# Oscar-W-Chen/gpu-ai-inference-server

Measured on AMD Instinct MI355X. Metric: images/sec, DenseNet-121 fp32, batch 32 per GPU, device-resident inputs, higher is better.
Workload: dtype f32; 1 GPU; DenseNet-121 fp32 batch=32 per GPU, synthetic 3x224x224 inputs (BASELINE configs[1]); synthetic ONNX graph + seeded random weights (reference model file is not in the mount); global_batch=32, per_gpu_batch=32, parallelism=dp1 (independent batch shards)

## Files before the change

gpu-ai-inference-server_amd/csrc/kernels_direct.hip:

```cpp
#include <hip/hip_runtime.h>

#include <algorithm>
#include <cstdlib>

#include "env.h"
#include "kernels.h"

namespace ie {

typedef float f32x16 __attribute__((ext_vector_type(16)));
typedef float f32x4 __attribute__((ext_vector_type(4)));
typedef float f32x2 __attribute__((ext_vector_type(2)));
typedef unsigned u32x4 __attribute__((ext_vector_type(4)));
typedef _Float16 h8 __attribute__((ext_vector_type(8)));
typedef _Float16 h2 __attribute__((ext_vector_type(2)));

struct DirectGeom {
    int cpt;
    int total;
};

template <bool HALF, int TN, int WAVES, int MAXC, bool PRE>
__global__ __launch_bounds__(64 * WAVES) void conv_direct_kernel(const ConvArgs a, const DirectGeom g) {
    constexpr int NT = 64 * WAVES, BN = 32 * TN;
    constexpr int CW = HALF ? 32 : 16;
    constexpr int ESZ = HALF ? 2 : 4;
    constexpr int PP = BN + 4;
    constexpr unsigned OOB = 0x80000000u;
    extern __shared__ __attribute__((aligned(16))) unsigned char smem_direct[];
    float* const sPart = reinterpret_cast<float*>(smem_direct);
    unsigned char* const sPre = smem_direct + size_t(WAVES) * 32 * PP * 4;

    const int tid = threadIdx.x, lane = tid & 63, r = lane & 31, hh = lane >> 5;
    const int wave = __builtin_amdgcn_readfirstlane(tid >> 6);
    const int Cin = a.in.c, H = a.in.h, W = a.in.w, OH = a.out.h, OW = a.out.w, Cout = a.out.c;
    const int M = a.out.n * OH * OW;
    const int m0 = blockIdx.x * 32, n0 = blockIdx.y * BN;
    const int KK = a.kh * a.kw;

    const int m = m0 + r;
    const bool mok = m < M;
    const int mm = mok ? m : 0;
    const int b = mm / (OH * OW);
    const int rem = mm - b * (OH * OW);
    const int oy = rem / OW, ox = rem - oy * OW;
    const int iy0 = oy * a.sh - a.pt, ix0 = ox * a.sw - a.pl;

    const int cb = int(int64_t(g.total) * wave / WAVES), ce = int(int64_t(g.total) * (wave + 1) / WAVES);
    const __amdgpu_buffer_rsrc_t rs_in = __builtin_amdgcn_make_buffer_rsrc(a.in.p, 0, int(a.in_bytes), 0x00020000);
    const void* const wbase = HALF ? a.w16 : static_cast<const void*>(a.w);
    const __amdgpu_buffer_rsrc_t rs_w = __builtin_amdgcn_make_buffer_rsrc(const_cast<void*>(wbase), 0, Cout * KK * Cin * ESZ, 0x00020000);

    u32x4 A[MAXC][2], B[MAXC][TN][2];
    unsigned okmask = 0;
#pragma unroll
    for (int i = 0; i < MAXC; ++i) {
        const int ch = cb + i;
        const bool live = ch < ce;
        const int chc = live ? ch : cb;
        const int tap = chc / g.cpt, c0 = (chc - tap * g.cpt) * CW;
        const int ky = tap / a.kw, kx = tap - ky * a.kw;
        const int iy = iy0 + ky, ix = ix0 + kx;
        const bool ok = live && mok && unsigned(iy) < unsigned(H) && unsigned(ix) < unsigned(W);
        okmask |= ok ? (1u << i) : 0u;
        const unsigned offA = ok ? unsigned(int(b * a.in.sn + iy * a.in.sh + ix * a.in.sw) + c0 + hh * (CW / 4)) * unsigned(ESZ) : OOB;
        A[i][0] = __builtin_amdgcn_raw_buffer_load_b128(rs_in, offA, 0, 0);
        A[i][1] = __builtin_amdgcn_raw_buffer_load_b128(rs_in, offA + unsigned(CW / 2 * ESZ), 0, 0);
#pragma unroll
        for (int j = 0; j < TN; ++j) {
            const int n = n0 + j * 32 + r;
            const unsigned offB = (live && n < Cout) ? unsigned((n * KK + tap) * Cin + c0 + hh * (CW / 4)) * unsigned(ESZ) : OOB;
            B[i][j][0] = __builtin_amdgcn_raw_buffer_load_b128(rs_w, offB, 0, 0);
            B[i][j][1] = __builtin_amdgcn_raw_buffer_load_b128(rs_w, offB + unsigned(CW / 2 * ESZ), 0, 0);
        }
    }

    if constexpr (PRE) {
        if constexpr (HALF) {
            const u32x4* const ps = static_cast<const u32x4*>(a.pre_scale16);
            const u32x4* const pt = static_cast<const u32x4*>(a.pre_shift16);
            u32x4* const ds = reinterpret_cast<u32x4*>(sPre);
            u32x4* const dt = reinterpret_cast<u32x4*>(sPre + Cin * 2);
            for (int i = tid; i < Cin / 8; i += NT) { ds[i] = ps[i]; dt[i] = pt[i]; }
        } else {
            const u32x4* const ps = reinterpret_cast<const u32x4*>(a.pre_scale);
            const u32x4* const pt = reinterpret_cast<const u32x4*>(a.pre_shift);
            u32x4* const ds = reinterpret_cast<u32x4*>(sPre);
            u32x4* const dt = reinterpret_cast<u32x4*>(sPre + Cin * 4);
            for (int i = tid; i < Cin / 4; i += NT) { ds[i] = ps[i]; dt[i] = pt[i]; }
        }
        __syncthreads();
    }

    f32x16 acc[TN];
#pragma unroll
    for (int j = 0; j < TN; ++j)
#pragma unroll
        for (int e = 0; e < 16; ++e) acc[j][e] = 0.f;

#pragma unroll
    for (int i = 0; i < MAXC; ++i) {
        if (cb + i < ce) {
            const int ch = cb + i;
            const int tap = ch / g.cpt, c0 = (ch - tap * g.cpt) * CW;
            const bool ok = (okmask >> i) & 1u;
#pragma unroll
            for (int q = 0; q < 2; ++q) {
                if constexpr (HALF) {
                    h8 av = __builtin_bit_cast(h8, A[i][q]);
                    if constexpr (PRE) {
                        const h8 s = *reinterpret_cast<const h8*>(sPre + (c0 + q * 16 + hh * 8) * 2);
                        const h8 t = *reinterpret_cast<const h8*>(sPre + Cin * 2 + (c0 + q * 16 + hh * 8) * 2);
                        av = av * s + t;
                        if (a.pre_relu) av = __builtin_elementwise_max(av, h8{});
                        if (!ok) av = h8{};
                    }
#pragma unroll
                    for (int j = 0; j < TN; ++j)
                        acc[j] = __builtin_amdgcn_mfma_f32_32x32x16_f16(__builtin_bit_cast(h8, B[i][j][q]), av, acc[j], 0, 0, 0);
                } else {
                    f32x4 av = __builtin_bit_cast(f32x4, A[i][q]);
                    if constexpr (PRE) {
                        const f32x4 s = *reinterpret_cast<const f32x4*>(sPre + (c0 + q * 8 + hh * 4) * 4);
                        const f32x4 t = *reinterpret_cast<const f32x4*>(sPre + Cin * 4 + (c0 + q * 8 + hh * 4) * 4);
#pragma unroll
                        for (int e = 0; e < 4; ++e) {
                            const float x = av[e] * s[e] + t[e];
                            av[e] = ok ? (a.pre_relu ? fmaxf(x, 0.f) : x) : 0.f;
                        }
                    }
#pragma unroll
                    for (int j = 0; j < TN; ++j) {
                        const f32x4 bv = __builtin_bit_cast(f32x4, B[i][j][q]);
#pragma unroll
                        for (int e = 0; e < 4; ++e) acc[j] = __builtin_amdgcn_mfma_f32_32x32x2f32(bv[e], av[e], acc[j], 0, 0, 0);
                    }
                }
            }
        }
    }

    float* const mine = sPart + (wave * 32 + r) * PP;
#pragma unroll
    for (int j = 0; j < TN; ++j)
#pragma unroll
        for (int gq = 0; gq < 4; ++gq)
            *reinterpret_cast<f32x4*>(mine + j * 32 + 8 * gq + 4 * hh) = f32x4{acc[j][4 * gq], acc[j][4 * gq + 1], acc[j][4 * gq + 2], acc[j][4 * gq + 3]};
    __syncthreads();
    const int esz = a.out.f16 ? 2 : 4;
    const __amdgpu_buffer_rsrc_t rs_out =
        __builtin_amdgcn_make_buffer_rsrc(a.out.p, 0, int((int64_t(M - 1) * a.out.sw + Cout) * esz), 0x00020000);
    for (int idx = tid; idx < 32 * (BN / 2); idx += NT) {
        const int p = idx / (BN / 2), c2 = (idx - p * (BN / 2)) * 2;
        f32x2 v = {0.f, 0.f};
#pragma unroll
        for (int w = 0; w < WAVES; ++w) {
            const f32x2 x = *reinterpret_cast<const f32x2*>(sPart + (w * 32 + p) * PP + c2);
            v[0] += x[0];
            v[1] += x[1];
        }
        const int n = n0 + c2;
        if (a.bias != nullptr) {
            v[0] += a.bias[n < Cout ? n : Cout - 1];
            v[1] += a.bias[n + 1 < Cout ? n + 1 : Cout - 1];
        }
        if (a.relu) { v[0] = fmaxf(v[0], 0.f); v[1] = fmaxf(v[1], 0.f); }
        const bool pok = m0 + p < M;
        const unsigned rowoff = pok ? unsigned((m0 + p) * int(a.out.sw) * esz) : OOB;
        if (a.out.f16) {
            const h2 hv = {_Float16(v[0]), _Float16(v[1])};
            __builtin_amdgcn_raw_buffer_store_b32(__builtin_bit_cast(unsigned, hv), rs_out, n < Cout ? rowoff + unsigned(n * 2) : OOB, 0, 0);
        } else {
            __builtin_amdgcn_raw_buffer_store_b64(__builtin_bit_cast(__attribute__((ext_vector_type(2))) unsigned, v), rs_out,
                                                  n < Cout ? rowoff + unsigned(n * 4) : OOB, 0, 0);
        }
    }
}

template <int TN, int WAVES, int MAXC, bool PRE>
__global__ __launch_bounds__(64 * WAVES) void conv_win_kernel(const ConvArgs a, const DirectGeom g) {
    constexpr int NT = 64 * WAVES, BN = 16 * TN, PP = BN + 4;
    constexpr unsigned OOB = 0x80000000u;
    extern __shared__ __attribute__((aligned(16))) unsigned char smem_direct[];
    float* const sWin = reinterpret_cast<float*>(smem_direct);
    float* const sPart = reinterpret_cast<float*>(smem_direct);

    const int tid = threadIdx.x, lane = tid & 63, r = lane & 15, gk = lane >> 4;
    const int wave = __builtin_amdgcn_readfirstlane(tid >> 6);
    const int Cin = a.in.c, H = a.in.h, W = a.in.w, Cout = a.out.c;
    const int P = Cin + 4;
    const int M = a.out.n * H * W;
    const int m0 = blockIdx.x * 16, n0 = blockIdx.y * BN;
    const int ipitch = int(a.in.sw);

    const int cb = int(int64_t(g.total) * wave / WAVES), ce = int(int64_t(g.total) * (wave + 1) / WAVES);
    const __amdgpu_buffer_rsrc_t rs_w =
        __builtin_amdgcn_make_buffer_rsrc(const_cast<float*>(a.wfrag), 0, Cout * a.kh * a.kw * Cin * 4, 0x00020000);
    u32x4 B[MAXC][TN];
#pragma unroll
    for (int i = 0; i < MAXC; ++i) {
        const int ch = cb + i;
#pragma unroll
        for (int j = 0; j < TN; ++j)
            B[i][j] = __builtin_amdgcn_raw_buffer_load_b128(
                rs_w, ch < ce ? unsigned(((int(blockIdx.y) * TN + j) * g.total + ch) * 64 + lane) * 16u : OOB, 0, 0);
    }

    {
        constexpr int U = 4;
        const __amdgpu_buffer_rsrc_t rs_in = __builtin_amdgcn_make_buffer_rsrc(a.in.p, 0, int(a.in_bytes), 0x00020000);
        const int c4n = Cin >> 2;
        const int p_lo = m0 - a.pt * W - a.pl;
        const int npx = 16 + (a.kh - 1) * W + (a.kw - 1);
        const int items = npx * c4n;
        for (int idx0 = tid; idx0 < items; idx0 += U * NT) {
            u32x4 v[U];
            int row[U], c4[U];
#pragma unroll
            for (int u = 0; u < U; ++u) {
                const int idx = idx0 + u * NT;
                row[u] = idx / c4n;
                c4[u] = idx - row[u] * c4n;
                const int p = p_lo + row[u];
                v[u] = __builtin_amdgcn_raw_buffer_load_b128(rs_in, (idx < items && p >= 0 && p < M) ? unsigned(p * ipitch + c4[u] * 4) * 4u : OOB, 0, 0);
            }
#pragma unroll
            for (int u = 0; u < U; ++u) {
                if (idx0 + u * NT < items) {
                    f32x4 x = __builtin_bit_cast(f32x4, v[u]);
                    if constexpr (PRE) {
                        const f32x4 sc = *reinterpret_cast<const f32x4*>(a.pre_scale + c4[u] * 4);
                        const f32x4 sf = *reinterpret_cast<const f32x4*>(a.pre_shift + c4[u] * 4);
#pragma unroll
                        for (int e = 0; e < 4; ++e) {
                            const float y = x[e] * sc[e] + sf[e];
                            x[e] = a.pre_relu ? fmaxf(y, 0.f) : y;
                        }
                    }
                    *reinterpret_cast<f32x4*>(sWin + row[u] * P + c4[u] * 4) = x;
                }
            }
        }
    }
    __syncthreads();

    const int m = m0 + r;
    const bool mok = m < M;
    const int rem = (mok ? m : 0) % (H * W);
    const int oy = rem / W, ox = rem - oy * W;

    f32x4 acc[TN];
#pragma unroll
    for (int j = 0; j < TN; ++j) acc[j] = f32x4{0.f, 0.f, 0.f, 0.f};
#pragma unroll
    for (int i = 0; i < MAXC; ++i) {
        if (cb + i < ce) {
            const int ch = cb + i;
            const int tap = ch / g.cpt, c0 = (ch - tap * g.cpt) * 16;
            const int ky = tap / a.kw, kx = tap - ky * a.kw;
            const bool ok = mok && unsigned(oy + ky - a.pt) < unsigned(H) && unsigned(ox + kx - a.pl) < unsigned(W);
            f32x4 av = *reinterpret_cast<const f32x4*>(sWin + (r + ky * W + kx) * P + c0 + gk * 4);
            if (!ok) av = f32x4{0.f, 0.f, 0.f, 0.f};
#pragma unroll
            for (int j = 0; j < TN; ++j) {
                const f32x4 bv = __builtin_bit_cast(f32x4, B[i][j]);
#pragma unroll
                for (int e = 0; e < 4; ++e) acc[j] = __builtin_amdgcn_mfma_f32_16x16x4f32(bv[e], av[e], acc[j], 0, 0, 0);
            }
        }
    }
    __syncthreads();

#pragma unroll
    for (int j = 0; j < TN; ++j) *reinterpret_cast<f32x4*>(sPart + (wave * 16 + r) * PP + j * 16 + 4 * gk) = acc[j];
    __syncthreads();
    const __amdgpu_buffer_rsrc_t rs_out =
        __builtin_amdgcn_make_buffer_rsrc(a.out.p, 0, int((int64_t(M - 1) * a.out.sw + Cout) * 4), 0x00020000);
    for (int idx = tid; idx < 16 * (BN / 2); idx += NT) {
        const int p = idx / (BN / 2), c2 = (idx - p * (BN / 2)) * 2;
        f32x2 v = {0.f, 0.f};
#pragma unroll
        for (int w = 0; w < WAVES; ++w) {
            const f32x2 x = *reinterpret_cast<const f32x2*>(sPart + (w * 16 + p) * PP + c2);
            v[0] += x[0];
            v[1] += x[1];
        }
        const int n = n0 + c2;
        if (a.bias != nullptr) { v[0] += a.bias[n]; v[1] += a.bias[n + 1]; }
        if (a.relu) { v[0] = fmaxf(v[0], 0.f); v[1] = fmaxf(v[1], 0.f); }
        __builtin_amdgcn_raw_buffer_store_b64(__builtin_bit_cast(__attribute__((ext_vector_type(2))) unsigned, v), rs_out,
                                              m0 + p < M ? unsigned((m0 + p) * int(a.out.sw) + n) * 4u : OOB, 0, 0);
    }
}

__global__ __launch_bounds__(256) void permute_weights_frag_kernel(const float* __restrict__ src, float* __restrict__ dst, int Cout, int KK, int Cin) {
    const int cpt = Cin >> 4, total = KK * cpt;
    const int64_t n4 = int64_t(Cout) * KK * Cin / 4;
    for (int64_t i = int64_t(blockIdx.x) * 256 + threadIdx.x; i < n4; i += int64_t(gridDim.x) * 256) {
        const int lane = int(i & 63);
        const int64_t t = i >> 6;
        const int ch = int(t % total), nb = int(t / total);
        const int tap = ch / cpt, c0 = (ch - tap * cpt) * 16;
        const int r = lane & 15, gk = lane >> 4;
        reinterpret_cast<f32x4*>(dst)[i] = *reinterpret_cast<const f32x4*>(src + (int64_t(nb * 16 + r) * KK + tap) * Cin + c0 + gk * 4);
    }
}

hipError_t LaunchPermuteWeightsFrag(const float* src, float* dst, int Cout, int KK, int Cin, hipStream_t stream) {
    if ((Cout % 16) || (Cin % 16) || Cout <= 0 || KK <= 0) return hipErrorInvalidValue;
    const int64_t n4 = int64_t(Cout) * KK * Cin / 4;
    const unsigned blocks = unsigned(std::min<int64_t>((n4 + 255) / 256, 2048));
    permute_weights_frag_kernel<<<dim3(blocks), dim3(256), 0, stream>>>(src, dst, Cout, KK, Cin);
    return hipGetLastError();
}

struct WinTile { int tn, waves, maxc; };
constexpr int kNumWinTiles = 4;
constexpr WinTile kWinTiles[kNumWinTiles] = {{1, 8, 9}, {2, 8, 9}, {1, 4, 18}, {2, 4, 18}};

static size_t win_lds_bytes(const ConvArgs& a, const WinTile& t) {
    const size_t win = size_t(16 + (a.kh - 1) * a.in.w + (a.kw - 1)) * (a.in.c + 4) * 4;
    const size_t part = size_t(t.waves) * 16 * (16 * t.tn + 4) * 4;
    return win > part ? win : part;
}

static bool win_eligible(const ConvArgs& a, int wt) {
    const WinTile t = kWinTiles[wt];
    if (a.in.f16 || a.out.f16 || a.wfrag == nullptr || a.res.p != nullptr) return false;
    if (a.in.sc != 1 || a.out.sc != 1 || (a.in.c % 16) || (a.out.c % (16 * t.tn))) return false;
    if (a.sh != 1 || a.sw != 1 || a.out.h != a.in.h || a.out.w != a.in.w || a.out.n != a.in.n) return false;
    if (a.pt < 0 || a.pl < 0 || a.pt >= a.kh || a.pl >= a.kw) return false;
    if ((a.in.sw % 4) || a.in.sh != a.in.w * a.in.sw || a.in.sn != a.in.h * a.in.sh || (reinterpret_cast<uintptr_t>(a.in.p) & 15)) return false;
    if ((reinterpret_cast<uintptr_t>(a.wfrag) & 15) || (a.out.sw & 1) || (reinterpret_cast<uintptr_t>(a.out.p) & 7)) return false;
    if (a.out.sh != a.out.w * a.out.sw || a.out.sn != a.out.h * a.out.sh) return false;
    if (a.pre_scale && ((reinterpret_cast<uintptr_t>(a.pre_scale) & 15) || (reinterpret_cast<uintptr_t>(a.pre_shift) & 15))) return false;
    const int64_t M = int64_t(a.out.n) * a.out.h * a.out.w;
    if (M > 65536 || (M + 64) * a.in.sw * 4 >= (int64_t(1) << 31) || M * a.out.sw * 4 >= (int64_t(1) << 31) ||
        int64_t(a.out.c) * a.kh * a.kw * a.in.c * 4 >= (int64_t(1) << 31))
        return false;
    const int total = a.kh * a.kw * (a.in.c / 16);
    if (total > t.waves * t.maxc || total < t.waves) return false;
    return win_lds_bytes(a, t) <= size_t(160) * 1024;
}

template <int WT>
static hipError_t launch_win_t(const ConvArgs& a, hipStream_t stream) {
    constexpr WinTile t = kWinTiles[WT];
    DirectGeom g;
    g.cpt = a.in.c / 16;
    g.total = a.kh * a.kw * g.cpt;
    const int64_t M = int64_t(a.out.n) * a.out.h * a.out.w;
    const dim3 grid(unsigned((M + 15) / 16), unsigned(a.out.c / (16 * t.tn)));
    const size_t lds = win_lds_bytes(a, t);
    if (a.pre_scale) conv_win_kernel<t.tn, t.waves, t.maxc, true><<<grid, dim3(64 * t.waves), lds, stream>>>(a, g);
    else conv_win_kernel<t.tn, t.waves, t.maxc, false><<<grid, dim3(64 * t.waves), lds, stream>>>(a, g);
    return hipGetLastError();
}

template <int WAVES, int TNW, int PB, bool PRE>
__global__ __launch_bounds__(64 * WAVES) void conv1x1_as_kernel(const ConvArgs a) {
    constexpr int NT = 64 * WAVES, D = PB == 1 ? 16 : 8, BNW = 16 * TNW, BN = BNW * WAVES;
    constexpr unsigned OOB = 0x80000000u;
    extern __shared__ __attribute__((aligned(16))) unsigned char smem_direct[];
    float* const sA = reinterpret_cast<float*>(smem_direct);

    const int tid = threadIdx.x, lane = tid & 63, r = lane & 15, gk = lane >> 4;
    const int wave = __builtin_amdgcn_readfirstlane(tid >> 6);
    const int K = a.in.c, P = K + (a.debug >> 8), CH = K >> 4, Cout = a.out.c;
    const int M = a.out.n * a.out.h * a.out.w;
    const int m0 = blockIdx.x * (16 * PB), n0 = blockIdx.y * BN + wave * BNW;
    const int ipitch = int(a.in.sw), opitch = int(a.out.sw);

    const __amdgpu_buffer_rsrc_t rs_w = __builtin_amdgcn_make_buffer_rsrc(const_cast<float*>(a.wfrag), 0, Cout * K * 4, 0x00020000);
    const int nb = n0 >> 4;
    u32x4 ring[D][TNW];
    int c_l = 0;
    const unsigned wlane = unsigned(lane) * 16u;
    auto issue = [&](int slot) {
        const int c = c_l < CH ? c_l : CH - 1;
#pragma unroll
        for (int j = 0; j < TNW; ++j) ring[slot][j] = __builtin_amdgcn_raw_buffer_load_b128(rs_w, wlane, ((nb + j) * CH + c) * 1024, 0);
        ++c_l;
    };
#pragma unroll
    for (int s = 0; s < D; ++s) issue(s);

    {
        constexpr int U = 4;
        const __amdgpu_buffer_rsrc_t rs_in = __builtin_amdgcn_make_buffer_rsrc(a.in.p, 0, int(a.in_bytes), 0x00020000);
        const int c4n = K >> 2;
        const int items = 16 * PB * c4n;
        for (int idx0 = tid; idx0 < items; idx0 += U * NT) {
            u32x4 v[U];
            int row[U], c4[U];
#pragma unroll
            for (int u = 0; u < U; ++u) {
                const int idx = idx0 + u * NT;
                row[u] = idx / c4n;
                c4[u] = idx - row[u] * c4n;
                const int p = m0 + row[u];
                v[u] = __builtin_amdgcn_raw_buffer_load_b128(rs_in, (idx < items && p < M) ? unsigned(p * ipitch + c4[u] * 4) * 4u : OOB, 0, 0);
            }
#pragma unroll
            for (int u = 0; u < U; ++u) {
                if (idx0 + u * NT < items) {
                    f32x4 x = __builtin_bit_cast(f32x4, v[u]);
                    if constexpr (PRE) {
                        const f32x4 sc = *reinterpret_cast<const f32x4*>(a.pre_scale + c4[u] * 4);
                        const f32x4 sf = *reinterpret_cast<const f32x4*>(a.pre_shift + c4[u] * 4);
#pragma unroll
                        for (int e = 0; e < 4; ++e) {
                            const float y = x[e] * sc[e] + sf[e];
                            x[e] = a.pre_relu ? fmaxf(y, 0.f) : y;
                        }
                    }
                    *reinterpret_cast<f32x4*>(sA + row[u] * P + c4[u] * 4) = x;
                }
            }
        }
    }
    __syncthreads();

    f32x4 acc[PB][TNW];
#pragma unroll
    for (int pb = 0; pb < PB; ++pb)
#pragma unroll
        for (int j = 0; j < TNW; ++j) acc[pb][j] = f32x4{0.f, 0.f, 0.f, 0.f};
    const float* abase[PB];
#pragma unroll
    for (int pb = 0; pb < PB; ++pb) abase[pb] = sA + (pb * 16 + r) * P + gk * 4;
    f32x4 avn[PB];
#pragma unroll
    for (int pb = 0; pb < PB; ++pb) avn[pb] = *reinterpret_cast<const f32x4*>(abase[pb]);
    auto compute = [&](int slot) {
        f32x4 av[PB];
#pragma unroll
        for (int pb = 0; pb < PB; ++pb) av[pb] = avn[pb];
#pragma unroll
        for (int pb = 0; pb < PB; ++pb) avn[pb] = *reinterpret_cast<const f32x4*>(abase[pb] + (slot + 1) * 16);
#pragma unroll
        for (int e = 0; e < 4; ++e)
#pragma unroll
            for (int j = 0; j < TNW; ++j)
#pragma unroll
                for (int pb = 0; pb < PB; ++pb)
                    acc[pb][j] = __builtin_amdgcn_mfma_f32_16x16x4f32(__builtin_bit_cast(f32x4, ring[slot][j])[e], av[pb][e], acc[pb][j], 0, 0, 0);
        __builtin_amdgcn_sched_group_barrier(0x100, PB, 0);
        __builtin_amdgcn_sched_group_barrier(0x008, 4 * PB * TNW, 0);
    };
    const int full = CH / D, rem = CH - full * D;
    for (int it = 0; it < full; ++it) {
#pragma unroll
        for (int s = 0; s < D; ++s) {
            compute(s);
            issue(s);
        }
#pragma unroll
        for (int pb = 0; pb < PB; ++pb) abase[pb] += D * 16;
    }
#pragma unroll
    for (int s = 0; s < D; ++s)
        if (s < rem) compute(s);

    const __amdgpu_buffer_rsrc_t rs_out =
        __builtin_amdgcn_make_buffer_rsrc(a.out.p, 0, int((int64_t(M - 1) * opitch + Cout) * 4), 0x00020000);
#pragma unroll
    for (int pb = 0; pb < PB; ++pb) {
        const int m = m0 + pb * 16 + r;
#pragma unroll
        for (int j = 0; j < TNW; ++j) {
            const int n = n0 + j * 16 + 4 * gk;
            f32x4 v = acc[pb][j];
            if (a.bias != nullptr) {
                const f32x4 bq = *reinterpret_cast<const f32x4*>(a.bias + n);
#pragma unroll
                for (int e = 0; e < 4; ++e) v[e] += bq[e];
            }
            if (a.relu) {
#pragma unroll
                for (int e = 0; e < 4; ++e) v[e] = fmaxf(v[e], 0.f);
            }
            __builtin_amdgcn_raw_buffer_store_b128(__builtin_bit_cast(u32x4, v), rs_out, m < M ? unsigned(m * opitch + n) * 4u : OOB, 0, 0);
        }
    }
}

struct AsTile { int waves, tnw, pb; };
constexpr int kNumAsTiles = 5;
constexpr AsTile kAsTiles[kNumAsTiles] = {{8, 1, 2}, {4, 1, 2}, {8, 2, 2}, {4, 1, 1}, {2, 2, 1}};

static bool as_eligible(const ConvArgs& a, int at) {
    const AsTile t = kAsTiles[at];
    if (a.in.f16 || a.out.f16 || a.wfrag == nullptr || a.res.p != nullptr) return false;
    if (a.kh != 1 || a.kw != 1 || a.sh != 1 || a.sw != 1 || a.pt != 0 || a.pl != 0) return false;
    if (a.out.h != a.in.h || a.out.w != a.in.w || a.out.n != a.in.n) return false;
    if (a.in.sc != 1 || a.out.sc != 1 || (a.in.c % 16) || (a.out.c % (16 * t.tnw * t.waves))) return false;
    if ((a.in.sw % 4) || a.in.sh != a.in.w * a.in.sw || a.in.sn != a.in.h * a.in.sh || (reinterpret_cast<uintptr_t>(a.in.p) & 15)) return false;
    if ((a.out.sw % 4) || a.out.sh != a.out.w * a.out.sw || a.out.sn != a.out.h * a.out.sh || (reinterpret_cast<uintptr_t>(a.out.p) & 15)) return false;
    if ((reinterpret_cast<uintptr_t>(a.wfrag) & 15) || (a.bias && (reinterpret_cast<uintptr_t>(a.bias) & 15))) return false;
    if (a.pre_scale && ((reinterpret_cast<uintptr_t>(a.pre_scale) & 15) || (reinterpret_cast<uintptr_t>(a.pre_shift) & 15))) return false;
    const int64_t M = int64_t(a.out.n) * a.out.h * a.out.w;
    if (M > (int64_t(1) << 22) || M * a.in.sw * 4 >= (int64_t(1) << 31) || M * a.out.sw * 4 >= (int64_t(1) << 31) || int64_t(a.out.c) * a.in.c * 4 >= (int64_t(1) << 31))
        return false;
    return size_t(16 * t.pb) * (a.in.c + 8) * 4 + 64 <= size_t(160) * 1024;
}

template <int AT>
static hipError_t launch_as_t(const ConvArgs& a_in, hipStream_t stream) {
    constexpr AsTile t = kAsTiles[AT];
    ConvArgs a = a_in;
    const int pad = Knobs().as_pad;
    a.debug = pad << 8;
    const int64_t M = int64_t(a.out.n) * a.out.h * a.out.w;
    const dim3 grid(unsigned((M + 16 * t.pb - 1) / (16 * t.pb)), unsigned(a.out.c / (16 * t.tnw * t.waves)));
    const size_t lds = size_t(16 * t.pb) * (a.in.c + pad) * 4 + 64;
    if (lds > size_t(160) * 1024) return hipErrorInvalidValue;
    if (a.pre_scale) conv1x1_as_kernel<t.waves, t.tnw, t.pb, true><<<grid, dim3(64 * t.waves), lds, stream>>>(a);
    else conv1x1_as_kernel<t.waves, t.tnw, t.pb, false><<<grid, dim3(64 * t.waves), lds, stream>>>(a);
    return hipGetLastError();
}

template <int AT>
static hipError_t init_as_t() {
    constexpr AsTile t = kAsTiles[AT];
    hipError_t e = hipFuncSetAttribute(reinterpret_cast<const void*>(&conv1x1_as_kernel<t.waves, t.tnw, t.pb, true>), hipFuncAttributeMaxDynamicSharedMemorySize, 160 * 1024);
    if (e != hipSuccess) return e;
    return hipFuncSetAttribute(reinterpret_cast<const void*>(&conv1x1_as_kernel<t.waves, t.tnw, t.pb, false>), hipFuncAttributeMaxDynamicSharedMemorySize, 160 * 1024);
}

struct DirectTile { int tn, waves, maxc; };
constexpr DirectTile kDirectTiles[kNumDirectBaseTiles] = {{1, 8, 8}, {1, 16, 4}, {1, 9, 8}, {1, 4, 8}, {1, 12, 6}, {2, 8, 4}};

static size_t direct_lds_bytes(int tile, int Cin, bool half, bool pre) {
    const DirectTile t = kDirectTiles[tile];
    return size_t(t.waves) * 32 * (32 * t.tn + 4) * 4 + (pre ? size_t(2) * Cin * (half ? 2 : 4) : 0);
}

bool ConvDirectEligible(const ConvArgs& a, int tile) {
    if (tile < 0 || tile >= kNumConvDirectTiles) return false;
    if (tile >= kNumDirectBaseTiles + kNumWinTiles) return as_eligible(a, tile - kNumDirectBaseTiles - kNumWinTiles);
    if (tile >= kNumDirectBaseTiles) return win_eligible(a, tile - kNumDirectBaseTiles);
    const bool half = a.in.f16 != 0;
    const int cw = half ? 32 : 16;
    if (a.in.sc != 1 || a.out.sc != 1 || (a.in.c % cw) || a.kh * a.kw > 49) return false;
    if (half ? (a.w16 == nullptr) : (a.w == nullptr)) return false;
    const int align = half ? 8 : 4;
    if ((a.in.sw % align) || (a.in.sh % align) || (a.in.sn % align) || (reinterpret_cast<uintptr_t>(a.in.p) & 15)) return false;
    if (reinterpret_cast<uintptr_t>(half ? a.w16 : static_cast<const void*>(a.w)) & 15) return false;
    if ((a.out.c & 1) || (a.out.sw & 1) || (reinterpret_cast<uintptr_t>(a.out.p) & 7)) return false;
    if (a.out.sh != a.out.w * a.out.sw || a.out.sn != a.out.h * a.out.sh) return false;
    if (a.pre_scale) {
        if (half && (a.pre_scale16 == nullptr || a.pre_shift16 == nullptr)) return false;
        if ((reinterpret_cast<uintptr_t>(a.pre_scale) & 15) || (reinterpret_cast<uintptr_t>(a.pre_shift) & 15)) return false;
        if (half && ((reinterpret_cast<uintptr_t>(a.pre_scale16) & 15) || (reinterpret_cast<uintptr_t>(a.pre_shift16) & 15))) return false;
    }
    const int esz = half ? 2 : 4;
    const int64_t in_span = int64_t(a.in.n - 1) * a.in.sn + int64_t(a.in.h - 1) * a.in.sh + int64_t(a.in.w - 1) * a.in.sw + a.in.c;
    const int64_t M = int64_t(a.out.n) * a.out.h * a.out.w;
    if (in_span * esz >= (int64_t(1) << 31) || M * a.out.sw * 4 >= (int64_t(1) << 31) ||
        int64_t(a.out.c) * a.kh * a.kw * a.in.c * esz >= (int64_t(1) << 31))
        return false;
    const DirectTile t = kDirectTiles[tile];
    const int total = a.kh * a.kw * (a.in.c / cw);
    if (total > t.waves * t.maxc || total < t.waves) return false;
    if (t.tn > 1 && a.out.c <= 32) return false;
    if (M > 65536) return false;
    return direct_lds_bytes(tile, a.in.c, half, a.pre_scale != nullptr) <= size_t(160) * 1024;
}

template <bool HALF, int T>
static hipError_t launch_direct_t(const ConvArgs& a, hipStream_t stream) {
    constexpr DirectTile t = kDirectTiles[T];
    DirectGeom g;
    g.cpt = a.in.c / (HALF ? 32 : 16);
    g.total = a.kh * a.kw * g.cpt;
    const int64_t M = int64_t(a.out.n) * a.out.h * a.out.w;
    const dim3 grid(unsigned((M + 31) / 32), unsigned((a.out.c + 32 * t.tn - 1) / (32 * t.tn)));
    const size_t lds = direct_lds_bytes(T, a.in.c, HALF, a.pre_scale != nullptr);
    if (a.pre_scale) conv_direct_kernel<HALF, t.tn, t.waves, t.maxc, true><<<grid, dim3(64 * t.waves), lds, stream>>>(a, g);
    else conv_direct_kernel<HALF, t.tn, t.waves, t.maxc, false><<<grid, dim3(64 * t.waves), lds, stream>>>(a, g);
    return hipGetLastError();
}

hipError_t LaunchConvDirect(const ConvArgs& a_in, int tile, hipStream_t stream) {
    if (!ConvDirectEligible(a_in, tile)) return hipErrorInvalidValue;
    ConvArgs a = a_in;
    const int esz = a.in.f16 ? 2 : 4;
    a.in_bytes = esz * (int64_t(a.in.n - 1) * a.in.sn + int64_t(a.in.h - 1) * a.in.sh + int64_t(a.in.w - 1) * a.in.sw + int64_t(a.in.c - 1) + 1);
    switch (tile - kNumDirectBaseTiles) {
        case 0: return launch_win_t<0>(a, stream);
        case 1: return launch_win_t<1>(a, stream);
        case 2: return launch_win_t<2>(a, stream);
        case 3: return launch_win_t<3>(a, stream);
        case 4: return launch_as_t<0>(a, stream);
        case 5: return launch_as_t<1>(a, stream);
        case 6: return launch_as_t<2>(a, stream);
        case 7: return launch_as_t<3>(a, stream);
        case 8: return launch_as_t<4>(a, stream);
        default: break;
    }
#define IE_DIR(T) \
    case T: return a.in.f16 ? launch_direct_t<true, T>(a, stream) : launch_direct_t<false, T>(a, stream);
    switch (tile) {
        IE_DIR(0) IE_DIR(1) IE_DIR(2) IE_DIR(3) IE_DIR(4) IE_DIR(5)
        default: return hipErrorInvalidValue;
    }
#undef IE_DIR
}

template <bool HALF, int T>
static hipError_t init_direct_t() {
    constexpr DirectTile t = kDirectTiles[T];
    hipError_t e = hipFuncSetAttribute(reinterpret_cast<const void*>(&conv_direct_kernel<HALF, t.tn, t.waves, t.maxc, true>),
                                       hipFuncAttributeMaxDynamicSharedMemorySize, 160 * 1024);
    if (e != hipSuccess) return e;
    return hipFuncSetAttribute(reinterpret_cast<const void*>(&conv_direct_kernel<HALF, t.tn, t.waves, t.maxc, false>),
                               hipFuncAttributeMaxDynamicSharedMemorySize, 160 * 1024);
}

template <int WT>
static hipError_t init_win_t() {
    constexpr WinTile t = kWinTiles[WT];
    hipError_t e = hipFuncSetAttribute(reinterpret_cast<const void*>(&conv_win_kernel<t.tn, t.waves, t.maxc, true>), hipFuncAttributeMaxDynamicSharedMemorySize, 160 * 1024);
    if (e != hipSuccess) return e;
    return hipFuncSetAttribute(reinterpret_cast<const void*>(&conv_win_kernel<t.tn, t.waves, t.maxc, false>), hipFuncAttributeMaxDynamicSharedMemorySize, 160 * 1024);
}

hipError_t InitKernelsDirect() {
    hipError_t e;
    if ((e = init_win_t<0>()) != hipSuccess) return e;
    if ((e = init_win_t<1>()) != hipSuccess) return e;
    if ((e = init_win_t<2>()) != hipSuccess) return e;
    if ((e = init_win_t<3>()) != hipSuccess) return e;
    if ((e = init_as_t<0>()) != hipSuccess) return e;
    if ((e = init_as_t<1>()) != hipSuccess) return e;
    if ((e = init_as_t<2>()) != hipSuccess) return e;
    if ((e = init_as_t<3>()) != hipSuccess) return e;
    if ((e = init_as_t<4>()) != hipSuccess) return e;
#define IE_DIRI(T)                                                     \
    if ((e = init_direct_t<false, T>()) != hipSuccess) return e;       \
    if ((e = init_direct_t<true, T>()) != hipSuccess) return e;
    IE_DIRI(0) IE_DIRI(1) IE_DIRI(2) IE_DIRI(3) IE_DIRI(4) IE_DIRI(5)
#undef IE_DIRI
    return hipSuccess;
}

}
```

Measured before the change: 14830 images/sec.

## Restructure 1x1 conv A-tile staging with column-blocked loads and specialized epilogue

Replaces the division-based flat staging loop of the 1x1 conv kernel with a column-blocked scheme: each thread owns a fixed column chunk, advances pointers incrementally, and issues grouped buffer loads whose width is chosen on the host via a new as_col_shift heuristic. Some weight prefetches are deferred until after staging. The pre-scale ReLU and the bias/ReLU epilogue become compile-time specializations, with bias hoisted per column tile. The intent is to cut integer address arithmetic and per-element branching in staging and epilogue, and to overlap weight loads with input staging. The cost is more code variants and possible OOB behaviour differences for partial row tiles that rely on the buffer range limit.

Result: faster. 15640 images/sec, median of 6 (+5.5%).

```diff
diff --git a/gpu-ai-inference-server_amd/csrc/kernels_direct.hip b/gpu-ai-inference-server_amd/csrc/kernels_direct.hip
--- a/gpu-ai-inference-server_amd/csrc/kernels_direct.hip
+++ b/gpu-ai-inference-server_amd/csrc/kernels_direct.hip
@@ -2,6 +2,7 @@
 
 #include <algorithm>
 #include <cstdlib>
+#include <type_traits>
 
 #include "env.h"
 #include "kernels.h"
@@ -360,13 +361,12 @@
 template <int WAVES, int TNW, int PB, bool PRE>
 __global__ __launch_bounds__(64 * WAVES) void conv1x1_as_kernel(const ConvArgs a) {
     constexpr int NT = 64 * WAVES, D = PB == 1 ? 16 : 8, BNW = 16 * TNW, BN = BNW * WAVES;
-    constexpr unsigned OOB = 0x80000000u;
     extern __shared__ __attribute__((aligned(16))) unsigned char smem_direct[];
     float* const sA = reinterpret_cast<float*>(smem_direct);
 
-    const int tid = threadIdx.x, lane = tid & 63, r = lane & 15, gk = lane >> 4;
+    const int tid = threadIdx.x;
     const int wave = __builtin_amdgcn_readfirstlane(tid >> 6);
-    const int K = a.in.c, P = K + (a.debug >> 8), CH = K >> 4, Cout = a.out.c;
+    const int K = a.in.c, P = K + ((a.debug >> 8) & 0xff), CH = K >> 4, Cout = a.out.c;
     const int M = a.out.n * a.out.h * a.out.w;
     const int m0 = blockIdx.x * (16 * PB), n0 = blockIdx.y * BN + wave * BNW;
     const int ipitch = int(a.in.sw), opitch = int(a.out.sw);
@@ -375,52 +375,84 @@
     const int nb = n0 >> 4;
     u32x4 ring[D][TNW];
     int c_l = 0;
-    const unsigned wlane = unsigned(lane) * 16u;
+    unsigned wlane = unsigned(tid & 63) * 16u;
     auto issue = [&](int slot) {
         const int c = c_l < CH ? c_l : CH - 1;
 #pragma unroll
         for (int j = 0; j < TNW; ++j) ring[slot][j] = __builtin_amdgcn_raw_buffer_load_b128(rs_w, wlane, ((nb + j) * CH + c) * 1024, 0);
         ++c_l;
     };
-#pragma unroll
-    for (int s = 0; s < D; ++s) issue(s);
+    constexpr int DLATE = D / 4;
+#pragma unroll
+    for (int s = 0; s < D - DLATE; ++s) issue(s);
 
     {
-        constexpr int U = 4;
-        const __amdgpu_buffer_rsrc_t rs_in = __builtin_amdgcn_make_buffer_rsrc(a.in.p, 0, int(a.in_bytes), 0x00020000);
-        const int c4n = K >> 2;
-        const int items = 16 * PB * c4n;
-        for (int idx0 = tid; idx0 < items; idx0 += U * NT) {
-            u32x4 v[U];
-            int row[U], c4[U];
-#pragma unroll
-            for (int u = 0; u < U; ++u) {
-                const int idx = idx0 + u * NT;
-                row[u] = idx / c4n;
-                c4[u] = idx - row[u] * c4n;
-                const int p = m0 + row[u];
-                v[u] = __builtin_amdgcn_raw_buffer_load_b128(rs_in, (idx < items && p < M) ? unsigned(p * ipitch + c4[u] * 4) * 4u : OOB, 0, 0);
-            }
-#pragma unroll
-            for (int u = 0; u < U; ++u) {
-                if (idx0 + u * NT < items) {
-                    f32x4 x = __builtin_bit_cast(f32x4, v[u]);
+        constexpr int R = 16 * PB, U = 4;
+        static_assert(R * 16 >= NT, "the narrowest column block (16 columns) must not span more rows than the tile has");
+        const int cs = a.debug >> 16, CT = 1 << cs;
+        const int rstep = NT >> cs, npass = R / rstep;
+        const int col = tid & (CT - 1), row0 = tid >> cs;
+        const __amdgpu_buffer_rsrc_t rs_in = __builtin_amdgcn_make_buffer_rsrc(a.in.p, 0, ((M - 1) * ipitch + K) * 4, 0x00020000);
+        const __amdgpu_buffer_rsrc_t rs_sc = __builtin_amdgcn_make_buffer_rsrc(const_cast<float*>(a.pre_scale), 0, PRE ? K * 4 : 0, 0x00020000);
+        const __amdgpu_buffer_rsrc_t rs_sf = __builtin_amdgcn_make_buffer_rsrc(const_cast<float*>(a.pre_shift), 0, PRE ? K * 4 : 0, 0x00020000);
+        const unsigned c16 = unsigned(col) * 16u;
+        unsigned g = (unsigned(m0) * unsigned(ipitch) + __umul24(row0, ipitch)) * 4u + c16;
+        unsigned char* l = smem_direct + (__umul24(row0, P) * 4u + c16);
+        const unsigned gstep = unsigned(rstep * ipitch) * 4u;
+        const unsigned gnext = unsigned(CT) * 16u - unsigned(npass) * gstep;
+        const int lstep = rstep * P * 4, lnext = CT * 16 - npass * lstep;
+        const f32x4 zero = {0.f, 0.f, 0.f, 0.f};
+        auto stage = [&](auto relu_) {
+            constexpr bool RELU = decltype(relu_)::value;
+            for (int left = K * 4; left > 0; left -= CT * 16) {
+                if (c16 < unsigned(left)) {
+                    f32x4 sc = zero, sf = zero;
                     if constexpr (PRE) {
-                        const f32x4 sc = *reinterpret_cast<const f32x4*>(a.pre_scale + c4[u] * 4);
-                        const f32x4 sf = *reinterpret_cast<const f32x4*>(a.pre_shift + c4[u] * 4);
-#pragma unroll
-                        for (int e = 0; e < 4; ++e) {
-                            const float y = x[e] * sc[e] + sf[e];
-                            x[e] = a.pre_relu ? fmaxf(y, 0.f) : y;
+                        sc = __builtin_bit_cast(f32x4, __builtin_amdgcn_raw_buffer_load_b128(rs_sc, c16, K * 4 - left, 0));
+                        sf = __builtin_bit_cast(f32x4, __builtin_amdgcn_raw_buffer_load_b128(rs_sf, c16, K * 4 - left, 0));
+                    }
+                    auto group = [&](auto n_) {
+                        constexpr int N = decltype(n_)::value;
+                        asm volatile("; ie-mark as-stage n=%0 relu=%1" ::"n"(N), "n"(int(RELU)));
+                        u32x4 v[N];
+#pragma unroll
+                        for (int u = 0; u < N; ++u) {
+                            v[u] = __builtin_amdgcn_raw_buffer_load_b128(rs_in, g, 0, 0);
+                            g += gstep;
                         }
+#pragma unroll
+                        for (int u = 0; u < N; ++u) {
+                            f32x4 x = __builtin_bit_cast(f32x4, v[u]);
+                            if constexpr (PRE) x = __builtin_elementwise_fma(x, sc, sf);
+                            if constexpr (PRE && RELU) x = __builtin_elementwise_max(x, zero);
+                            *reinterpret_cast<f32x4*>(l) = x;
+                            l += lstep;
+                        }
+                        asm volatile("; ie-mark as-stage-end n=%0 relu=%1" ::"n"(N), "n"(int(RELU)));
+                    };
+                    if (npass >= U) {
+                        for (int p0 = 0; p0 < npass; p0 += U) group(std::integral_constant<int, U>{});
+                    } else if (npass == 2) {
+                        group(std::integral_constant<int, 2>{});
+                    } else {
+                        group(std::integral_constant<int, 1>{});
                     }
-                    *reinterpret_cast<f32x4*>(sA + row[u] * P + c4[u] * 4) = x;
+                    g += gnext;
+                    l += lnext;
                 }
             }
-        }
-    }
+        };
+        if (PRE && __builtin_amdgcn_readfirstlane(a.pre_relu) != 0) stage(std::true_type{});
+        else stage(std::false_type{});
+    }
+#pragma unroll
+    for (int s = D - DLATE; s < D; ++s) issue(s);
     __syncthreads();
 
+    int lane = __builtin_amdgcn_mbcnt_hi(~0u, __builtin_amdgcn_mbcnt_lo(~0u, 0u));
+    asm volatile("" : "+v"(lane));
+    const int r = lane & 15, gk = lane >> 4;
+    wlane = unsigned(lane) * 16u;
     f32x4 acc[PB][TNW];
 #pragma unroll
     for (int pb = 0; pb < PB; ++pb)
@@ -428,7 +460,7 @@
         for (int j = 0; j < TNW; ++j) acc[pb][j] = f32x4{0.f, 0.f, 0.f, 0.f};
     const float* abase[PB];
 #pragma unroll
-    for (int pb = 0; pb < PB; ++pb) abase[pb] = sA + (pb * 16 + r) * P + gk * 4;
+    for (int pb = 0; pb < PB; ++pb) abase[pb] = sA + (__umul24(r, P) + pb * 16 * P + gk * 4);
     f32x4 avn[PB];
 #pragma unroll
     for (int pb = 0; pb < PB; ++pb) avn[pb] = *reinterpret_cast<const f32x4*>(abase[pb]);
@@ -464,24 +496,31 @@
 
     const __amdgpu_buffer_rsrc_t rs_out =
         __builtin_amdgcn_make_buffer_rsrc(a.out.p, 0, int((int64_t(M - 1) * opitch + Cout) * 4), 0x00020000);
-#pragma unroll
-    for (int pb = 0; pb < PB; ++pb) {
-        const int m = m0 + pb * 16 + r;
+    const __amdgpu_buffer_rsrc_t rs_b = __builtin_amdgcn_make_buffer_rsrc(const_cast<float*>(a.bias), 0, a.bias != nullptr ? Cout * 4 : 0, 0x00020000);
+    const unsigned o0 = (unsigned(m0) * unsigned(opitch) + __umul24(r, opitch) + 4 * gk) * 4u;
+    const unsigned ostep = unsigned(opitch) * 64u;
+    const f32x4 zero = {0.f, 0.f, 0.f, 0.f};
+    auto finish = [&](auto relu_, auto bias_) {
+        constexpr bool RELU = decltype(relu_)::value, BIAS = decltype(bias_)::value;
+        asm volatile("; ie-mark as-finish relu=%0 bias=%1" ::"n"(int(RELU)), "n"(int(BIAS)));
 #pragma unroll
         for (int j = 0; j < TNW; ++j) {
-            const int n = n0 + j * 16 + 4 * gk;
-            f32x4 v = acc[pb][j];
-            if (a.bias != nullptr) {
-                const f32x4 bq = *reinterpret_cast<const f32x4*>(a.bias + n);
-#pragma unroll
-                for (int e = 0; e < 4; ++e) v[e] += bq[e];
+            f32x4 bq = zero;
+            if constexpr (BIAS) bq = __builtin_bit_cast(f32x4, __builtin_amdgcn_raw_buffer_load_b128(rs_b, unsigned(gk) * 16u, (n0 + j * 16) * 4, 0));
+#pragma unroll
+            for (int pb = 0; pb < PB; ++pb) {
+                f32x4 v = acc[pb][j];
+                if constexpr (BIAS) v += bq;
+                if constexpr (RELU) v = __builtin_elementwise_max(v, zero);
+                __builtin_amdgcn_raw_buffer_store_b128(__builtin_bit_cast(u32x4, v), rs_out, o0 + pb * ostep, (n0 + j * 16) * 4, 0);
             }
-            if (a.relu) {
-#pragma unroll
-                for (int e = 0; e < 4; ++e) v[e] = fmaxf(v[e], 0.f);
-            }
-            __builtin_amdgcn_raw_buffer_store_b128(__builtin_bit_cast(u32x4, v), rs_out, m < M ? unsigned(m * opitch + n) * 4u : OOB, 0, 0);
-        }
+        }
+    };
+    switch (__builtin_amdgcn_readfirstlane((a.relu ? 1 : 0) | (a.bias != nullptr ? 2 : 0))) {
+        case 0: finish(std::false_type{}, std::false_type{}); break;
+        case 1: finish(std::true_type{}, std::false_type{}); break;
+        case 2: finish(std::false_type{}, std::true_type{}); break;
+        default: finish(std::true_type{}, std::true_type{}); break;
     }
 }
 
@@ -502,7 +541,20 @@
     const int64_t M = int64_t(a.out.n) * a.out.h * a.out.w;
     if (M > (int64_t(1) << 22) || M * a.in.sw * 4 >= (int64_t(1) << 31) || M * a.out.sw * 4 >= (int64_t(1) << 31) || int64_t(a.out.c) * a.in.c * 4 >= (int64_t(1) << 31))
         return false;
+    if (a.in.sw >= (int64_t(1) << 22) || a.out.sw >= (int64_t(1) << 22)) return false;
     return size_t(16 * t.pb) * (a.in.c + 8) * 4 + 64 <= size_t(160) * 1024;
+}
+
+static int as_col_shift(int K, int threads, int rows) {
+    const int c4n = K / 4;
+    int best = 6;
+    long best_key = -1;
+    for (int s = 6; s >= 4; --s) {
+        const int ct = 1 << s, blocks = (c4n + ct - 1) / ct, npass = rows * ct / threads;
+        const long key = (long(blocks * ((npass + 3) / 4)) << 24) + blocks * npass;
+        if (best_key < 0 || key < best_key) best = s, best_key = key;
+    }
+    return best;
 }
 
 template <int AT>
@@ -510,7 +562,7 @@
     constexpr AsTile t = kAsTiles[AT];
     ConvArgs a = a_in;
     const int pad = Knobs().as_pad;
-    a.debug = pad << 8;
+    a.debug = (pad << 8) | (as_col_shift(a.in.c, 64 * t.waves, 16 * t.pb) << 16);
     const int64_t M = int64_t(a.out.n) * a.out.h * a.out.w;
     const dim3 grid(unsigned((M + 16 * t.pb - 1) / (16 * t.pb)), unsigned(a.out.c / (16 * t.tnw * t.waves)));
     const size_t lds = size_t(16 * t.pb) * (a.in.c + pad) * 4 + 64;
```
